# JuliaMolSim/Molly.jl

Hardware: AMD Instinct MI355X
Metric: ns_per_day (higher is better)
Workload: dtype f32; 1 GPU; 1M-atom LJ fluid (argon, rho=21.1/nm3), cubic PBC, DistanceCutoff 1.0 nm, r_list 1.2 nm, dt 2 fs, VelocityVerlet, remove_CM_motion=1; integrator=vv, n_atoms=1000000, rebuild_every=10, parallelism=single domain, block_atoms=256, j_split=2, pairs_half_list=75841147

## Files before the change

### molly.jl_amd/csrc/engine.hip

```cpp
#include <algorithm>
#include <chrono>
#include <cstddef>
#include <cstdlib>
#include <cstring>
#include <limits>
#include <memory>
#include <new>
#include <string>
#include <vector>

#include <unistd.h>

#include "bonded.h"
#include "stochastic.h"
#include "constraints.h"
#include "virtual_sites.h"
#include "pme.h"
#include "step_fused.h"
#include "hilbert.h"
#include "kernels.h"
#include "list_policy.h"
#include "replan.h"
#include "halo_step.h"
#include "forces_launch.h"
// ... 742 lines not shown
        bool step = false;
        bool gcv = false;
        bool cm = false, measure = false;
        double dt = 0;
        const StochP<T>* lang = nullptr;
        bool halo = false, halo_cm_in = false;
        bool fuse_spread = false, fuse_terms = false;
        const double* cm_sum_in = nullptr;
        T4* frc = nullptr;
    };
    struct PassRes {
        bool step = false; int parts = 0;
        bool gs = false, spread = false, terms = false;
        bool cm_summed = false;
    };
    bool packed_kind(bool energy) const {
        return std::is_same<T, float>::value && ljm == LJ_DIST_UNIFORM && coulm == MHIP_COUL_NONE && !energy && !minimg && n_special == 0 && eshift == ESHIFT_SCALED && I.lj_c12 != T(0);
    }
    int packed_stride(int tile_max, bool energy) const {
        if (!packed_kind(energy) || segmented) return 0;
        for (int k = 0; k < 3; ++k) if (tile_max + 1 < SOA_STRIDES[k]) return SOA_STRIDES[k];
        return 0;
    }
    PassRes launch_pair_kernel(bool energy, int part = 0, bool allow_gs = false, const PassReq& req = PassReq{}) {
        PassRes res;
        prune_resolve(!(xf_direct && n_ghost > 0));
        ForceArgs<T> A;
        A.G = G; A.I = I; A.n_owned = n_owned; A.BI = BI; A.BI_shift = ilog2(BI); A.JS = JS; A.T_cap = T_cap; A.T_lds = tile_lds; A.R_cap = R_cap;
        A.n_blocks = n_blocks; A.blocks_per_xcd = cdiv(n_blocks, 8);
        A.orig = nullptr; A.S = StochP<T>{};
        A.pos = pos[cur].p; A.lj = lj[cur].p; A.tile_idx = tile_idx.p; A.tile_cnt = tile_cnt.p;
        if constexpr (std::is_same<T, float>::value) {
            if (dual && !inner_valid && !energy && allow_gs && part == 0 && !req.frc && adopt_env && gs_groups() > 0 && cnt_outer_valid && margin_zero && !(lp.skin_in < lp.skin)
                && lp.last_outer_step == pass_step && n_ghost == 0 && !host_prune) adopt_outer_list();
        }
        const bool use_inner = dual && inner_valid;
        const bool prune = dual && !inner_valid && !energy;
        const int GS = gs_groups();
        if constexpr (std::is_same<T, float>::value) {
            if (allow_gs && GS > 0 && use_inner && !energy && part == 0 && gs_list_id == n_filters && !req.frc) {
                const int q_lds = (max_tile_in + GS - 1) / GS + 1;
                if (gs_lds_bytes(q_lds, BI, JS / GS) <= (size_t)MAX_LDS_BYTES / GS) {
                    frc_parts.reserve((size_t)(GS - 1) * cap);
                    GsArgs Z;
                    Z.G = G; Z.I = I; Z.n_owned = n_owned; Z.BI = BI; Z.BI_shift = ilog2(BI); Z.JS = JS; Z.GS = GS; Z.lgGS = ilog2(GS); Z.R_cap = GS * R_cap;
                     Z.T_cap = T_cap; Z.Q_lds = q_lds;
// ... 17 lines not shown
                                                  reinterpret_cast<const BondedArgs<float>&>(static_cast<const BondedArgs<T>&>(bonded.slot_args(G, I, pos[cur].p, inv.p))), cdiv(bonded.n_blocks(), 4), lds, stream,
                                                  gs_cm_fin ? pending_cm.parts_arg() : (const double*)nullptr, pending_cm.n, gs_cm_fin ? cm_fin_buf.p : (double*)nullptr);
                        if (gs_cm_fin) pending_cm.moved(cm_fin_buf.p, 1);
                        res.spread = with_spread; res.terms = !with_spread;
                    } else launch_forces_gs(Z, coulm, minimg, stream);
                    prof.end(0, stream);
                    MHIP_HIP(hipGetLastError());
                    ++n_force_calls; ++n_gs_passes; res.gs = true;
                    if (Z.dbg && (n_gs_passes % stamps_every()) == 0) stamps_dump("", (size_t)n_blocks * GS * 4 * 8);
                    return res;
                }
            }
        }
        const size_t prune_extra = prune ? prune_lds_bytes(std::min(T_cap, max_tile + 1), BI * JS) + 16 : 0;
        carve_force_lds(use_inner ? max_tile_in : max_tile, prune_extra);
        last_pass_tile = use_inner ? max_tile_in : max_tile;
        A.T_lds = tile_lds;
        if (use_inner && !inner_is_outer) { A.tile_idx = tile_idx_in.p; A.tile_cnt = tile_cnt_in.p; }
        A.nbr = (use_inner && !inner_is_outer) ? nbr_in.p : nbr.p; A.wave_rows = (use_inner && !inner_is_outer) ? wave_rows_in.p : wave_rows.p;
        A.nbr_dst = nullptr; A.rows_dst = nullptr; A.pos_snap = nullptr; A.blk_disp2 = nullptr; A.r_prune2 = r_prune2;
        A.tile_idx_dst = nullptr; A.tile_cnt_dst = nullptr; A.mark_off = 0; A.snap_dst = nullptr; A.any_special = n_special > 0 ? 1 : 0; A.eshift = eshift;
        A.cnt_dst = nullptr;
        A.soa = packed_stride(use_inner ? max_tile_in : max_tile, energy);
        if (A.soa) lds_force = std::max((size_t)3 * A.soa * sizeof(float) + 64, (size_t)JS * 4 * BI * sizeof(T) + 32);
        A.part = 0; A.blk_ghost = nullptr;
        if (part != 0 && !prune) {
            DBuf<int32_t>& fl = use_inner ? blk_ghost_in : blk_ghost; bool& ok = use_inner ? ghost_flags_in_ok : ghost_flags_ok;
            if (!ok) {
                fl.reserve(n_blocks);
                hipLaunchKernelGGL(k_block_ghost_flags, dim3(n_blocks), dim3(WAVE), 0, stream, n_blocks, T_cap, n_owned, (const int32_t*)A.tile_idx, (const int32_t*)A.tile_cnt, fl.p);
                ok = true;
            }
            A.part = part; A.blk_ghost = fl.p;
        }
        if (prune) {
            wave_rows_in.reserve((size_t)n_blocks * JS * (BI / WAVE)); nbr_in.reserve((size_t)n_blocks * JS * R_cap * BI); blk_disp2.reserve((size_t)n_blocks * (BI / WAVE));
            A.nbr_dst = nbr_in.p; A.rows_dst = wave_rows_in.p; A.pos_snap = pos_snap.p; A.blk_disp2 = blk_disp2.p;
            pos_snap_in.reserve(cap);
            A.snap_dst = pos_snap_in.p;
            if (n_ghost > 0) MHIP_HIP(hipMemcpyAsync(pos_snap_in.p + n_owned, pos[cur].p + n_owned, (size_t)n_ghost * sizeof(T4), hipMemcpyDeviceToDevice, stream));
            lp.last_prune_step = pass_step;
            tile_idx_in.reserve((size_t)n_blocks * T_cap); tile_cnt_in.reserve(n_blocks);
            A.tile_idx_dst = tile_idx_in.p; A.tile_cnt_dst = tile_cnt_in.p;
            inner_is_outer = false;
            if (GS > 0) { cnt_in.reserve((size_t)n_blocks * JS * BI); A.cnt_dst = cnt_in.p; }
            A.mark_off = (int)((lds_force + 15) & ~(size_t)15);
            if (A.soa && A.mark_off != prune_mark_ct(A.soa)) throw ApiError{MHIP_ERR_STATE, "internal: the packed pruning pass expects its renumbering table at " + std::to_string(prune_mark_ct(A.soa)) + ", the carve-up put it at " + std::to_string(A.mark_off)};
            lds_force = (size_t)A.mark_off + prune_lds_bytes(tile_lds, BI * JS);
            if (lds_force > (size_t)MAX_LDS_BYTES) throw ApiError{MHIP_ERR_CAPACITY, "prune pass LDS carve-up exceeds 160 KiB"};
        }
        A.blk_center = blk_center.p; A.frc = req.frc ? req.frc : frc[cur].p; A.pe_part = red_part.p;
        A.cm_fin_in = nullptr; A.cm_fin_n = 0; A.cm_fin_out = nullptr;
        A.vel = nullptr; A.pos_next = nullptr; A.dt = T(0); A.dt2 = T(0); A.cm_in = nullptr; A.cm_n = 0; A.cm_pub = nullptr; A.step_seq = 0; A.cm_out = nullptr; A.trk_part = nullptr; A.snap_a = nullptr; A.snap_b = nullptr;
        const bool cm_fin = (in_vv_fused || in_lang_fused) && !energy && n_ghost == 0 && part == 0 && pending_cm.mode() == 2 && pending_cm.n > 1 && pending_cm.n <= 65536;
        if (cm_fin) { cm_fin_buf.reserve(4); A.cm_fin_in = pending_cm.parts_arg(); A.cm_fin_n = pending_cm.n; A.cm_fin_out = cm_fin_buf.p; }
        else if (req.cm_sum_in && !energy && n_ghost == 0 && part == 0) {
            cm_fin_buf.reserve(4); A.cm_fin_in = req.cm_sum_in; A.cm_fin_n = pending_cm.n; A.cm_fin_out = cm_fin_buf.p; res.cm_summed = true;
        }
        A.level_pairs = (prune && JS == 2) ? 1 : 0;
        A.dbg = (!prune && !energy) ? stamps_begin((size_t)n_blocks * 16 * 8) : nullptr;
        bool do_step = false;
        if constexpr (std::is_same<T, float>::value) {
            do_step = req.step && fuse_step_env && A.soa != 0 && use_inner && !prune && part == 0 && !req.frc && (n_ghost == 0 || req.halo) && pending_cm.mode() != 1;
            if (req.halo && !do_step) throw ApiError{MHIP_ERR_STATE, "internal: the fused ghosted step was asked for a pass that cannot integrate"};
            if (do_step) {
                pos_alt.reserve(cap); cm_blk.reserve(2 * 4 * (size_t)n_blocks + 8);
                if (!cm_pub.p) { cm_pub.reserve(4); MHIP_HIP(hipMemsetAsync(cm_pub.p, 0, 4 * sizeof(unsigned long long), stream)); }
                A.vel = vel[cur].p; A.pos_next = pos_alt.p; A.dt = T(req.dt); A.dt2 = T(req.dt) / T(2);
                A.cm_in = pending_cm.parts_arg(); A.cm_n = pending_cm.n; A.cm_pub = cm_pub.p; A.step_seq = ++step_seq;
                A.cm_out = req.cm ? cm_blk.p + (size_t)step_half * 4 * n_blocks : (double*)nullptr;
                A.trk_part = nullptr; A.snap_a = pos_snap_in.p; A.snap_b = pos_snap.p;
// ... 33 lines not shown
        prof.end(prune ? 4 : 0, stream);
        MHIP_HIP(hipGetLastError());
        ++n_force_calls;
        if (A.dbg && (n_force_calls % stamps_every()) == 0) stamps_report();
        if (prune) {
            const bool late = xf_direct && n_ghost > 0 && prune_late_env;
            if (late) { h_prune.make(N_FLAGS); ev_prune.make(hipEventDisableTiming); }
            int32_t* const h_dst = late ? h_prune : h_flags;
            hipLaunchKernelGGL(k_prune_summary, dim3(1), dim3(1024), 0, stream, n_blocks, n_blocks * JS * (BI / WAVE), n_blocks * (BI / WAVE), R_cap,
                               (const int32_t*)tile_cnt_in.p, wave_rows_in.p, (const float*)blk_disp2.p, flags.p, h_dst);
            if (n_ghost > 0) {
                hipLaunchKernelGGL(k_max_disp<T>, dim3(std::min(cdiv(n_ghost, 256), 1024)), dim3(256), 0, stream, n_ghost, (const T4*)pos[cur].p + n_owned, (const T4*)pos_snap.p + n_owned,
                                   reinterpret_cast<unsigned int*>(flags.p + FLAG_MAX_DISP2), G);
                MHIP_HIP(hipMemcpyAsync(h_dst, flags.p, N_FLAGS * sizeof(int32_t), hipMemcpyDeviceToHost, stream));
            }
            ++n_filters; ghost_flags_in_ok = false; lp.next_check_step = -1; hx.tile_ok = false; hx.trk_step = -1;
            inner_valid = true;
            if (late) {
                MHIP_HIP(hipEventRecord(ev_prune, stream));
                prune_pending = true; prune_pending_id = n_filters; prune_disp_exceeded = false;
                max_tile_in = max_tile;
            } else {
                MHIP_HIP(hipStreamSynchronize(stream));
                prune_pending = false;
                float d2; std::memcpy(&d2, &h_flags[FLAG_MAX_DISP2], sizeof(float));
                total_rows = h_flags[FLAG_TOTAL_ROWS]; max_tile_in = h_flags[FLAG_MAX_TILE];
                prune_disp_exceeded = !lp.prune_stands(std::sqrt((double)d2));
                if (debug_on) std::fprintf(stderr, "[mhip] prune: max disp %.5f nm (margin %.3f) rows %lld exceeded %d calls %lld\n", std::sqrt((double)d2), lp.prune_margin(), (long long)total_rows, (int)prune_disp_exceeded, (long long)n_force_calls);
            }
        }
        return res;
    }

    DBuf<double> cm_fin_buf;
    int step_half = 0;
    uint32_t step_seq = 0;
    int64_t n_fused_steps = 0;
    int step_parts = 0;
    const bool fuse_gcv_env = env_int("MOLLYHIP_FUSE_GATHER_VV", 1) != 0;
    DBuf<T4> pos_alt; DBuf<double> cm_blk; DBuf<unsigned long long> cm_pub;
    const bool fuse_step_env = env_int("MOLLYHIP_FUSE_STEP", 1) != 0;
    const bool halo_waiter_env = env_int("MOLLYHIP_HALO_WAITER", 1) != 0;
    const bool prune_late_env = env_int("MOLLYHIP_PRUNE_LATE", 1) != 0;
    bool packed_step_possible() {
        if (!fuse_step_env || !dual || !inner_valid || stale || !packed_kind(false)) return false;
        prune_resolve(false);
        if (prune_pending && max_tile_in + 1 >= SOA_STRIDES[2]) prune_resolve(true);
        if (max_tile_in + 1 >= SOA_STRIDES[2]) return false;
        carve_force_lds(max_tile_in);
        return packed_stride(max_tile_in, false) != 0;
    }
// ... 1820 lines not shown
```

### molly.jl_amd/csrc/kernels.h

```cpp
#pragma once
#include <type_traits>
#include "physics.h"
#include "halo_xfer.h"
#include "philox.h"

namespace mhip {

enum { FLAG_MINIMG = 0, FLAG_OVERFLOW = 1, FLAG_MAX_TILE = 2, FLAG_MAX_ROWS = 3, FLAG_NAN = 4, FLAG_TOTAL_ROWS = 5, FLAG_MAX_CELLS = 6, FLAG_MAX_DISP2 = 7, FLAG_MAX_V2 = 8, N_FLAGS = 10 };
enum { OVF_TILE = 1, OVF_ROWS = 2, OVF_BOXCELLS = 4, OVF_SLOT = 8 };

constexpr int MAX_BOX_CELLS = 8192;
constexpr uint32_t XL_EXCLUDED = 1u << 30, XL_SPECIAL = 1u << 31, XL_INDEX = (1u << 30) - 1u;

constexpr int ESHIFT_SCALED = 2;
constexpr int SLOT_MAX_SCALED = 16383;
__host__ __device__ inline uint32_t entry_slot(uint32_t e, int sh) { return sh ? (e >> sh) : (e & 0x7fffu); }
__host__ __device__ inline uint32_t entry_special(uint32_t e, int sh) { return sh ? 0u : (e >> 15); }
__host__ __device__ inline uint32_t make_entry(uint32_t slot, uint32_t sp, int sh) { return sh ? (slot << sh) : (slot | (sp << 15)); }

template <class T> __device__ inline int cell_coord(T x, int d, const GridP<T>& G) {
    T rel = G.periodic[d] ? x : x - G.origin[d];
    int c = (int)M<T>::floor(rel * G.inv_cs[d]);
    return min(max(c, 0), G.nc[d] - 1);
}

extern "C" __device__ int mhip_writelane_i32(int src, int lane, int old) __asm("llvm.amdgcn.writelane.i32");
__device__ inline void mask_to_lane(int& lo, int& hi, unsigned long long mask, int dst) {
// ... 1086 lines not shown
#pragma unroll
    for (int o = 32; o > 0; o >>= 1) for (int c = 0; c < 4; ++c) a[c] += __shfl_xor(a[c], o, 64);
    if ((threadIdx.x & 63) == 0) for (int c = 0; c < 4; ++c) sh_pub[threadIdx.x >> 6][c] = a[c];
    __syncthreads();
    if (threadIdx.x < 3) {
        double t = 0, m = 0;
        for (int q = 0; q < (int)(blockDim.x >> 6); ++q) { t += sh_pub[q][threadIdx.x]; m += sh_pub[q][3]; }
        const float vc = (float)(t / m);
        __hip_atomic_store(&pub[threadIdx.x], (unsigned long long)__float_as_uint(vc) | ((unsigned long long)seq << 32), __ATOMIC_RELAXED, __HIP_MEMORY_SCOPE_AGENT);
    }
}
[[maybe_unused]] static __device__ inline void cm_finalize_in_block(const double* __restrict__ part, int n_part, double* out4, unsigned char* smem) {
    double a[4] = {0, 0, 0, 0};
    for (int q = threadIdx.x; q < n_part; q += blockDim.x) { const double* p = part + 4 * (int64_t)q; a[0] += p[0]; a[1] += p[1]; a[2] += p[2]; a[3] += p[3]; }
#pragma unroll
    for (int o = 32; o > 0; o >>= 1) for (int c = 0; c < 4; ++c) a[c] += __shfl_xor(a[c], o, 64);
    double* sh = reinterpret_cast<double*>(smem);
    if ((threadIdx.x & 63) == 0) for (int c = 0; c < 4; ++c) sh[4 * (threadIdx.x >> 6) + c] = a[c];
    __syncthreads();
    if (threadIdx.x < 4) { double t = 0; for (int q = 0; q < (int)(blockDim.x >> 6); ++q) t += sh[4 * q + threadIdx.x]; out4[threadIdx.x] = t; }
    __syncthreads();
}
constexpr int SOA_STRIDES[3] = {2049, 3073, 4097};
__host__ __device__ constexpr int prune_mark_ct(int soa) { return (3 * soa * 4 + 64 + 15) & ~15; }
__host__ __device__ inline size_t prune_lds_bytes(int t_seg, int nthr) { return (size_t)(((t_seg + 8) & ~7) * 2) + ((size_t)nthr + 4) * 4 + 8 * 8 * 4 + ((size_t)nthr + 64) * 4 + 16 * 8 + 32; }

#ifndef MHIP_FAST_MIN_WAVES
#define MHIP_FAST_MIN_WAVES 8
#endif
#ifndef MHIP_SB
#define MHIP_SB 4
#endif
template <class T, int LJM, int COULM, bool ENERGY, bool MINIMG, bool SEG, bool PRUNE>
constexpr int force_min_waves() { return (std::is_same<T, float>::value && LJM == LJ_DIST_UNIFORM && COULM == MHIP_COUL_NONE && !ENERGY && !MINIMG && !SEG && !PRUNE) ? MHIP_FAST_MIN_WAVES : 1; }

template <class T, int LJM, int COULM, bool ENERGY, bool MINIMG, bool SEG, bool PRUNE, int SOA_STRIDE = 4097, bool STEP = false, bool HALO = false, bool LANG = false>
__global__ void __launch_bounds__(BlockLimits<T>::max_threads, (force_min_waves<T, LJM, COULM, ENERGY, MINIMG, SEG, PRUNE>()))
k_forces(ForceArgs<T> A) {
    static_assert(!HALO || (STEP && std::is_same<T, float>::value), "the ghosted form exists for the fused fp32 step only");
    static_assert(!LANG || (STEP && !HALO), "the Langevin update rides in the fused single-domain step only");
    using T4 = typename Vec<T>::T4;
    using T2 = typename Vec<T>::T2;
    constexpr bool PER_ATOM_LJ = (LJM == LJ_DIST || LJM == LJ_GENERIC);
    extern __shared__ __align__(32) unsigned char smem[];
    const GridP<T>& G = A.G;
    int wg = blockIdx.x;
    if constexpr (STEP) {
        if (wg == 0) {
            if constexpr (HALO) { if (A.cm_in) halo_cm_publish(A.H, A.cm_pub, A.step_seq, smem); }
            else if (A.cm_in) step_cm_publish(A.cm_in, A.cm_n, A.cm_pub, A.step_seq, smem);
            return;
        }
        --wg;
    }
    int b = (wg & 7) * A.blocks_per_xcd + (wg >> 3);
    [[maybe_unused]] int hflags = 0;
    if constexpr (HALO) { b = A.H.order[wg]; if (b < 0) return; hflags = A.H.flags[b]; }
// ... 41 lines not shown
    int rows = 0;
    bool own_done = false;
    auto own_ready = [&]() {
        if (own_done) return;
        own_done = true;
        if constexpr (NO_TRI) pi = localise(pi_raw, std::false_type{});
        else pi = tri_local ? localise(pi_raw, std::true_type{}) : localise(pi_raw, std::false_type{});
        lji = pre_e(lji_raw);
        rows = __builtin_amdgcn_readfirstlane(rows_lane);
    };
    if constexpr (PRUNE) own_ready();
    const uint2* my_rows = A.nbr + (((int64_t)b * A.JS + js) * A.R_cap) * A.BI + li;
    const int32_t* tix = (HALO ? A.H.tsrc : A.tile_idx) + (int64_t)b * A.T_cap;
    if constexpr (HALO) { if (hflags & 1) halo_wait_block(A.H); }
    T fx = T(0), fy = T(0), fz = T(0), pe = T(0);
    [[maybe_unused]] T vir[6] = {T(0), T(0), T(0), T(0), T(0), T(0)};
    uint64_t acc = 0;
    int kept = 0;
    uint2* out_rows = nullptr;
    if constexpr (PRUNE) out_rows = A.nbr_dst + (((int64_t)b * A.JS + js) * A.R_cap) * A.BI + li;
    [[maybe_unused]] uint16_t* l_new = nullptr; [[maybe_unused]] int32_t* l_scan = nullptr; [[maybe_unused]] float* l_box = nullptr;
    [[maybe_unused]] int32_t* l_cnt = nullptr; [[maybe_unused]] int32_t* l_wmax = nullptr; [[maybe_unused]] const uint2* l_lut = nullptr;
    [[maybe_unused]] int n_new = 0;
    if constexpr (PRUNE) {
        l_new = reinterpret_cast<uint16_t*>(smem + A.mark_off);
        l_scan = reinterpret_cast<int32_t*>(smem + A.mark_off + ((A.T_lds + 8) & ~7) * 2);
        l_box = reinterpret_cast<float*>(l_scan + nthr + 4);
        l_wmax = reinterpret_cast<int32_t*>(l_box + 64); l_cnt = l_wmax + 64;
        if (tid < 64) l_wmax[tid] = 0;
        l_lut = reinterpret_cast<const uint2*>(l_cnt + nthr);
        if (tid < 16) {
            uint32_t sel[2] = {0x0c0c0c0cu, 0x0c0c0c0cu};
            int p = 0;
            for (int j = 0; j < 4; ++j) if ((tid >> j) & 1) {
                const int sh = (p & 1) * 16;
                sel[p >> 1] = (sel[p >> 1] & ~(0xffffu << sh)) | ((uint32_t)((2 * j) | ((2 * j + 1) << 8)) << sh);
                ++p;
            }
            reinterpret_cast<uint2*>(l_cnt + nthr)[tid] = make_uint2(sel[0], sel[1]);
        }
        const int lpb = A.BI >> 3;
        float mn[3] = {(float)pi.x, (float)pi.y, (float)pi.z}, mx[3] = {(float)pi.x, (float)pi.y, (float)pi.z};
        for (int o = lpb >> 1; o > 0; o >>= 1)
#pragma unroll
            for (int d = 0; d < 3; ++d) { mn[d] = fminf(mn[d], __shfl_xor(mn[d], o, WAVE)); mx[d] = fmaxf(mx[d], __shfl_xor(mx[d], o, WAVE)); }
        if (js == 0 && (li & (lpb - 1)) == 0) {
            reinterpret_cast<float4*>(l_box)[(li / lpb) * 2] = make_float4(mn[0], mn[1], mn[2], 0.f);
            reinterpret_cast<float4*>(l_box)[(li / lpb) * 2 + 1] = make_float4(mx[0], mx[1], mx[2], 0.f);
        }
        if (A.snap_dst && js == 0 && valid) A.snap_dst[si] = pi_raw;
    }
    [[maybe_unused]] auto emit4 = [&](uint32_t n0, uint32_t n1, uint32_t n2, uint32_t n3, bool k0, bool k1, bool k2, bool k3) {
        const uint32_t m = (k0 ? 1u : 0u) | (k1 ? 2u : 0u) | (k2 ? 4u : 0u) | (k3 ? 8u : 0u);
        const uint2 sel = l_lut[m];
        const uint32_t x = __builtin_amdgcn_perm(n1, n0, 0x05040100u), y = __builtin_amdgcn_perm(n3, n2, 0x05040100u);
        const uint64_t p = ((uint64_t)__builtin_amdgcn_perm(y, x, sel.y) << 32) | __builtin_amdgcn_perm(y, x, sel.x);
        const int np = kept & 3, sh = np * 16;
        const uint64_t c_lo = acc | (p << sh), c_hi = (p >> 1) >> (63 - sh);
        const int cnt = __builtin_popcount(m);
        const bool flush = np + cnt >= 4;
        if (flush) out_rows[(int64_t)(kept >> 2) * A.BI] = make_uint2((uint32_t)c_lo, (uint32_t)(c_lo >> 32));
        acc = flush ? c_hi : c_lo;
        kept += cnt;
    };
    auto emit = [&](uint32_t e) {
        const int np = kept & 3;
        acc |= (uint64_t)e << (np * 16);
        if (np == 3) { out_rows[(int64_t)(kept >> 2) * A.BI] = make_uint2((uint32_t)acc, (uint32_t)(acc >> 32)); acc = 0; }
        ++kept;
    };

    constexpr bool FAST_CT = std::is_same<T, float>::value && LJM == LJ_DIST_UNIFORM && COULM == MHIP_COUL_NONE && !ENERGY && !MINIMG && !SEG;
    const int seg_cap = A.T_lds;
// ... 11 lines not shown
                    for (int k = 0; k < SB; ++k) s[k] = tix[min(t0 + k * nthr + tid, A.T_cap - 1)];
#pragma unroll
                    for (int k = 0; k < SB; ++k) {
                        s[k] = (t0 + k * nthr + tid < n_here) ? s[k] : (int)((int64_t)b * A.BI);
                        if constexpr (HALO) {
                            if (s[k] >= 0) p[k] = A.pos[s[k]];
                            else { const float* gr = A.H.rows + 3 * (size_t)(-1 - s[k]); p[k] = make4<T>((T)peer_row_load(gr), (T)peer_row_load(gr + 1), (T)peer_row_load(gr + 2), T(0)); }
                        } else p[k] = A.pos[s[k]];
                    }
#pragma unroll
                    for (int k = 0; k < SB; ++k) {
                        const int t = t0 + k * nthr + tid;
                        if (t < n_here) {
                            const T4 pl = localise(p[k], tri_tag);
                            if (packed3) { l_p3[t] = (float)pl.x; l_p3[SOA_STRIDE + t] = (float)pl.y; l_p3[2 * SOA_STRIDE + t] = (float)pl.z; }
                            else l_pos[t] = pl;
                        }
                    }
                };
                round(0);
                for (int t0 = SB * nthr; t0 < n_here; t0 += SB * nthr) round(t0);
                return;
            }
            for (int t0 = 0; t0 < n_here; t0 += SB * nthr) {
                int s[SB]; T4 p[SB]; [[maybe_unused]] T2 q[SB];
                constexpr bool GUARD = !(FAST_CT && !PRUNE);
                const int kmax = GUARD ? min(SB, (n_here - t0 + nthr - 1) / nthr) : SB;
#pragma unroll
                for (int k = 0; k < SB; ++k) {
                    if (k < kmax) {
                        const int t = min(t0 + k * nthr + tid, n_here - 1);
                        s[k] = tix[seg_lo + t];
                    }
                }
#pragma unroll
                for (int k = 0; k < SB; ++k) if (k < kmax) { p[k] = A.pos[s[k]]; if constexpr (PER_ATOM_LJ) q[k] = A.lj[s[k]]; }
#pragma unroll
                for (int k = 0; k < SB; ++k) {
                    const int t = t0 + k * nthr + tid;
                    if (k < kmax && t < n_here) {
                        const T4 pl = localise(p[k], tri_tag);
                        if (packed3) { l_p3[t] = (float)pl.x; l_p3[SOA_STRIDE + t] = (float)pl.y; l_p3[2 * SOA_STRIDE + t] = (float)pl.z; }
                        else l_pos[t] = pl;
                        if constexpr (PER_ATOM_LJ) l_lj[t] = pre_e(q[k]);
                    }
                }
            }
        };
        if constexpr (NO_TRI) stage(std::false_type{});
        else { if (tri_local) stage(std::true_type{}); else stage(std::false_type{}); }
        own_ready();
        if (tid == 0) {
            if (packed3) { l_p3[n_here] = 1e4f; l_p3[SOA_STRIDE + n_here] = 1e4f; l_p3[2 * SOA_STRIDE + n_here] = 1e4f; }
            else l_pos[n_here] = make4<T>(T(1e4), T(1e4), T(1e4), T(0));
            if constexpr (PER_ATOM_LJ) l_lj[n_here] = make2<T>(T(0), T(0));
        }
        __syncthreads();
        if constexpr (PRUNE) {
            constexpr int NW = 8;
            const float reach2 = (float)A.r_prune2 * 1.001f + 1e-12f;
            const float bL[3] = {(float)G.L[0], (float)G.L[1], (float)G.L[2]}, biL[3] = {(float)G.invL[0], (float)G.invL[1], (float)G.invL[2]};
            auto stays = [&](int t) -> bool {
                if constexpr (MINIMG) { if (G.triclinic) return true; }
                float p[3];
                if (packed3) { p[0] = l_p3[t]; p[1] = l_p3[SOA_STRIDE + t]; p[2] = l_p3[2 * SOA_STRIDE + t]; }
                else { const T4 q = l_pos[t]; p[0] = (float)q.x; p[1] = (float)q.y; p[2] = (float)q.z; }
                float best = 3.0e38f;
#pragma unroll 1
                for (int w = 0; w < NW; ++w) {
                    const float4 lo = reinterpret_cast<const float4*>(l_box)[2 * w], hi = reinterpret_cast<const float4*>(l_box)[2 * w + 1];
                    float ex, ey, ez;
                    if constexpr (MINIMG) {
                        const float blo[3] = {lo.x, lo.y, lo.z}, bhi[3] = {hi.x, hi.y, hi.z};
                        float e[3];
#pragma unroll
                        for (int d = 0; d < 3; ++d) {
                            float dd = p[d] - 0.5f * (blo[d] + bhi[d]);
                            if (G.periodic[d]) dd -= bL[d] * rintf(dd * biL[d]);
                            e[d] = fmaxf(fabsf(dd) - 0.5f * (bhi[d] - blo[d]) - 1e-5f * bL[d], 0.f);
                        }
                        ex = e[0]; ey = e[1]; ez = e[2];
                    } else {
                        ex = fmaxf(fmaxf(lo.x - p[0], p[0] - hi.x), 0.f); ey = fmaxf(fmaxf(lo.y - p[1], p[1] - hi.y), 0.f); ez = fmaxf(fmaxf(lo.z - p[2], p[2] - hi.z), 0.f);
                    }
                    best = fminf(best, ex * ex + ey * ey + ez * ez);
                }
                return best <= reach2;
            };
            const int per = (n_here + nthr - 1) / nthr, t0 = min(tid * per, n_here), t1 = min(t0 + per, n_here);
            int cnt = 0;
            uint32_t keep_bits = 0;
            for (int t = t0; t < t1; ++t) { const bool k = stays(t); cnt += k ? 1 : 0; if (t - t0 < 32) keep_bits |= (k ? 1u : 0u) << (t - t0); }
            l_scan[tid] = cnt;
            __syncthreads();
            if (tid < WAVE) {
                int run = 0;
                for (int base = 0; base < nthr; base += WAVE) {
                    int v = (base + tid < nthr) ? l_scan[base + tid] : 0, x = v;
#pragma unroll
                    for (int o = 1; o < WAVE; o <<= 1) { int u = __shfl_up(x, o, WAVE); if (tid >= o) x += u; }
                    if (base + tid < nthr) l_scan[base + tid] = run + x - v;
                    run += __shfl(x, WAVE - 1, WAVE);
                }
                if (tid == 0) l_scan[nthr] = run;
            }
            __syncthreads();
            {
                int run = n_new + l_scan[tid];
                for (int t = t0; t < t1; ++t) {
                    if ((t - t0 < 32) ? ((keep_bits >> (t - t0)) & 1u) != 0u : stays(t)) { l_new[t] = (uint16_t)(packed3 ? run << ESHIFT_SCALED : run); A.tile_idx_dst[(int64_t)b * A.T_cap + run] = tix[seg_lo + t]; ++run; }
                    else l_new[t] = (uint16_t)0xffffu;
                }
            }
            n_new += l_scan[nthr];
            __syncthreads();
        }
        stamp(1);
        auto walk_rows = [&](auto spec_tag) {
            constexpr bool SPEC = decltype(spec_tag)::value;
            if constexpr (FAST_CT && !SPEC) { if (packed3) {
                typedef float v2f __attribute__((ext_vector_type(2)));
                const v2f pix = {(float)pi.x, (float)pi.x}, piy = {(float)pi.y, (float)pi.y}, piz = {(float)pi.z, (float)pi.z};
                const float c6 = (float)A.I.lj_c6, c12 = (float)A.I.lj_c12, rc2 = (float)A.I.lj_rc2, rp2 = (float)A.r_prune2;
                const float rc2n = __int_as_float(__float_as_int(rc2) + 1);
                const v2f cut_a = {-0x1p100f, -0x1p100f}, cut_b = {rc2n * 0x1p100f, rc2n * 0x1p100f};
                const v2f c48v = {c12, c12}, c24v = {c6, c6};
                v2f fx2 = {(float)fx, 0.f}, fy2 = {(float)fy, 0.f}, fz2 = {(float)fz, 0.f};
                typedef __attribute__((address_space(3))) const char* lds_cptr;
                const lds_cptr lbase = (lds_cptr)(uintptr_t)0;
                auto lds3 = [&](uint32_t oa, uint32_t ob, v2f& dx, v2f& dy, v2f& dz) {
                    typedef __attribute__((address_space(3))) const float* lds_fptr;
                    const lds_fptr pa = (lds_fptr)(lbase + oa), pb = (lds_fptr)(lbase + ob);
                    dx = (v2f){pa[0], pb[0]} - pix; dy = (v2f){pa[SOA_STRIDE], pb[SOA_STRIDE]} - piy; dz = (v2f){pa[2 * SOA_STRIDE], pb[2 * SOA_STRIDE]} - piz;
                };
                auto row = [&](const uint2 e4) {
                    const uint32_t oa = e4.x & 0xffffu, ob = e4.x >> 16, oc = e4.y & 0xffffu, od = e4.y >> 16;
                    v2f dx0, dy0, dz0, dx1, dy1, dz1;
                    lds3(oa, ob, dx0, dy0, dz0); lds3(oc, od, dx1, dy1, dz1);
                    __builtin_amdgcn_sched_group_barrier(0x100, 12, 0);
                    const v2f r20 = __builtin_elementwise_fma(dz0, dz0, __builtin_elementwise_fma(dy0, dy0, dx0 * dx0));
                    const v2f r21 = __builtin_elementwise_fma(dz1, dz1, __builtin_elementwise_fma(dy1, dy1, dx1 * dx1));
                    if constexpr (PRUNE) {
                        typedef __attribute__((address_space(3))) const unsigned short* lds_hptr;
                        auto new_entry = [&](uint32_t o) -> uint32_t { return (uint32_t)*(lds_hptr)(lbase + prune_mark_ct(SOA_STRIDE) + (o >> 1)); };
                        const uint32_t na = new_entry(oa), nb = new_entry(ob), nc = new_entry(oc), nd = new_entry(od);
                        emit4(na, nb, nc, nd, r20.x <= rp2, r20.y <= rp2, r21.x <= rp2, r21.y <= rp2);
                    }
                    const float t0 = __builtin_amdgcn_rcpf(r20.x * r20.y), t1 = __builtin_amdgcn_rcpf(r21.x * r21.y);
                    const v2f u0 = (v2f){r20.y, r20.x} * t0, u1 = (v2f){r21.y, r21.x} * t1;
                    v2f in0, in1;
                    asm("v_pk_fma_f32 %0, %1, %2, %3 clamp\n\ts_nop 0" : "=v"(in0) : "v"(r20), "s"(cut_a), "v"(cut_b));
                    asm("v_pk_fma_f32 %0, %1, %2, %3 clamp\n\ts_nop 0" : "=v"(in1) : "v"(r21), "s"(cut_a), "v"(cut_b));
                    const v2f q0 = u0 * u0, q1 = u1 * u1;
                    const v2f w0 = u0 * in0, w1 = u1 * in1;
                    const v2f c0 = q0 * u0, c1 = q1 * u1;
                    const v2f g0 = __builtin_elementwise_fma(c0, c48v, -c24v), g1 = __builtin_elementwise_fma(c1, c48v, -c24v);
                    const v2f h0 = c0 * w0, h1 = c1 * w1;
                    const v2f f0 = g0 * h0, f1 = g1 * h1;
                    fx2 -= dx0 * f0; fy2 -= dy0 * f0; fz2 -= dz0 * f0;
                    fx2 -= dx1 * f1; fy2 -= dy1 * f1; fz2 -= dz1 * f1;
                };
                if (rows > 0) {
                    const int last = rows - 1;
                    constexpr int D = 2;
                    uint2 e[D] = {my_rows[0], my_rows[(int64_t)min(1, last) * A.BI]};
                    auto next = [&](int q) -> uint2 { return my_rows[(int64_t)min(q, last) * A.BI]; };
                    int r = 0;
                    for (; r + D <= rows; r += D) {
#pragma unroll
// ... 94 lines not shown
            __syncthreads();
            const int kp = l_cnt[tid ^ A.BI], total = kept + kp, mine = js == 0 ? (total + 1) >> 1 : total >> 1;
            if (kept > mine) {
                uint16_t* to = reinterpret_cast<uint16_t*>(A.nbr_dst + (((int64_t)b * A.JS + (js ^ 1)) * A.R_cap) * A.BI + li);
                const uint16_t* from = reinterpret_cast<const uint16_t*>(out_rows);
                for (int q = 0; q < kept - mine; ++q) {
                    const int ps = mine + q, pd = kp + q;
                    to[(((int64_t)(pd >> 2) * A.BI) << 2) + (pd & 3)] = from[(((int64_t)(ps >> 2) * A.BI) << 2) + (ps & 3)];
                }
            }
            kept = mine;
        }
        if (A.cnt_dst) A.cnt_dst[((int64_t)b * A.JS + js) * A.BI + li] = (uint16_t)min(kept, 65535);
        atomicMax(&l_wmax[js * NWB + (li >> 6)], (kept + 3) >> 2);
        __syncthreads();
        const int rows_wave = l_wmax[js * NWB + (li >> 6)];
        if (level) {
            uint16_t* mine16 = reinterpret_cast<uint16_t*>(out_rows);
            for (int p2 = kept; p2 < 4 * rows_wave; ++p2) mine16[(((int64_t)(p2 >> 2) * A.BI) << 2) + (p2 & 3)] = (uint16_t)SENTP;
        } else
        while (((kept + 3) >> 2) < rows_wave || (kept & 3)) emit(SENTP);
        if (tid < A.JS * NWB) A.rows_dst[b * A.JS * NWB + tid] = l_wmax[tid];
        if (tid == 0) A.tile_cnt_dst[b] = n_new;
        float d2 = 0.f;
        if (valid && js == 0) {
            T4 q = A.pos_snap[si];
            T ex = pi_raw.x - q.x, ey = pi_raw.y - q.y, ez = pi_raw.z - q.z;
            disp_image(ex, ey, ez, G);
            d2 = (float)(ex * ex + ey * ey + ez * ez);
        }
        d2 = wave_max(d2);
        if (js == 0 && (tid & 63) == 0) A.blk_disp2[b * (A.BI >> 6) + (li >> 6)] = d2;
    }
    stamp(2);
    [[maybe_unused]] T4 st_v, st_p;
    [[maybe_unused]] int64_t se = 0;
    [[maybe_unused]] unsigned long long st_w[3] = {0, 0, 0};
    [[maybe_unused]] int snd0 = 0, snd1 = 0;
    if constexpr (STEP) {
        __builtin_amdgcn_s_setprio(3);
        se = step_atom();
        if constexpr (HALO) { if ((hflags & 2) && js == 0 && se < A.n_owned) { snd0 = A.H.snd_start[se]; snd1 = A.H.snd_start[se + 1]; } }
        if (js == 0 && se < A.n_owned) {
            st_v = A.vel[se]; st_p = A.pos[se];
            if (A.cm_in) {
#pragma unroll
                for (int c = 0; c < 3; ++c) st_w[c] = __hip_atomic_load(&A.cm_pub[c], __ATOMIC_RELAXED, __HIP_MEMORY_SCOPE_AGENT);
            }
        }
    }
    if (A.JS > 1) {
        __syncthreads();
// ... 79 lines not shown
            }
            if (A.trk_part && tid < 3) { float mm = 0.f; for (int q = 0; q < 4 * nw; ++q) mm = fmaxf(mm, shf[4 * q + tid]); A.trk_part[(int64_t)tid * A.n_blocks + b] = mm; }
        }
        if (mine) { A.vel[se] = v; A.pos_next[se] = p; }
        if constexpr (HALO) {
            if (js == 0) {
                if (hflags & 2) {
                    if (!(hflags & 1)) { const int ln = tid & 63; if (ln < A.H.n_peers && !xfer_wait(&A.H.seq_in[A.H.peers[ln]], A.H.seq_wait, A.H.err, A.H.ticks, (9 << 8) | A.H.peers[ln])) atomicOr(A.H.err, 1); }
                    if (mine) for (int r = snd0; r < snd1; ++r) {
                        const HaloSend e = A.H.snd[r];
                        float* d = e.dst + (int64_t)A.H.parity_send * A.H.half_stride;
                        __hip_atomic_store(d, (float)p.x + e.sx, __ATOMIC_RELAXED, __HIP_MEMORY_SCOPE_SYSTEM);
                        __hip_atomic_store(d + 1, (float)p.y + e.sy, __ATOMIC_RELAXED, __HIP_MEMORY_SCOPE_SYSTEM);
                        __hip_atomic_store(d + 2, (float)p.z + e.sz, __ATOMIC_RELAXED, __HIP_MEMORY_SCOPE_SYSTEM);
                    }
                }
                asm volatile("s_waitcnt vmcnt(0)" ::: "memory");
                unsigned int before = 0;
                if ((tid & 63) == 0) before = __hip_atomic_fetch_add(A.H.done, 1u, __ATOMIC_RELAXED, __HIP_MEMORY_SCOPE_AGENT);
                before = (unsigned int)__builtin_amdgcn_readfirstlane((int)before);
                if (before == A.H.n_done - 1u) halo_tail(A.H, A.cm_out, A.n_blocks);
            }
        }
    } else {
        if (js == 0 && valid) A.frc[si] = make4<T>(fx, fy, fz, T(0));
    }
    stamp(3);
    if constexpr (!ENERGY) {
        if (A.cm_fin_out && wg == 0) { __syncthreads(); cm_finalize_in_block(A.cm_fin_in, A.cm_fin_n, A.cm_fin_out, smem); }
    }
    if constexpr (ENERGY) {
        if (A.JS > 1) {
            T* red = reinterpret_cast<T*>(smem);
#pragma unroll
            for (int half = 0; half < 2; ++half) {
                __syncthreads();
#pragma unroll
                for (int c = 0; c < 3; ++c) red[(js * 4 + c) * A.BI + li] = vir[3 * half + c];
                __syncthreads();
                if (js == 0) for (int q = 1; q < A.JS; ++q) for (int c = 0; c < 3; ++c) vir[3 * half + c] += red[(q * 4 + c) * A.BI + li];
            }
        }
        __syncthreads();
        double* dred = reinterpret_cast<double*>(smem);
        for (int c = 0; c < 7; ++c) {
            if (js == 0) dred[li] = valid ? 0.5 * (double)(c == 0 ? pe : vir[c - 1]) : 0.0;
// ... 339 lines not shown
```

Measured before the change: 1372 ns/day.

## Compact pruning pass staging to a smaller LDS stride with box-distance filtering

Result: faster. 1413 ns/day (median of 6 runs) (+3.0%).

```diff
diff --git a/molly.jl_amd/csrc/engine.hip b/molly.jl_amd/csrc/engine.hip
--- a/molly.jl_amd/csrc/engine.hip
+++ b/molly.jl_amd/csrc/engine.hip
@@ -788,6 +788,11 @@
         for (int k = 0; k < 3; ++k) if (tile_max + 1 < SOA_STRIDES[k]) return SOA_STRIDES[k];
         return 0;
     }
+    int prune_kept_tile = -1;
+    static int prune_stride_for(int tile, int soa_outer) {
+        for (int k = 0; k < 3; ++k) if (tile + 1 < SOA_STRIDES[k]) return std::min(SOA_STRIDES[k], soa_outer);
+        return soa_outer;
+    }
     PassRes launch_pair_kernel(bool energy, int part = 0, bool allow_gs = false, const PassReq& req = PassReq{}) {
         PassRes res;
         prune_resolve(!(xf_direct && n_ghost > 0));
@@ -851,6 +856,9 @@
         A.tile_idx_dst = nullptr; A.tile_cnt_dst = nullptr; A.mark_off = 0; A.snap_dst = nullptr; A.any_special = n_special > 0 ? 1 : 0; A.eshift = eshift;
         A.cnt_dst = nullptr;
         A.soa = packed_stride(use_inner ? max_tile_in : max_tile, energy);
+        const bool prune_sync = prune && n_ghost == 0;
+        const int soa_outer = A.soa;
+        if (prune && A.soa && prune_sync && GS <= 0 && prune_kept_tile >= 0) A.soa = prune_stride_for(prune_kept_tile + prune_kept_tile / 128 + 4, soa_outer);
         if (A.soa) lds_force = std::max((size_t)3 * A.soa * sizeof(float) + 64, (size_t)JS * 4 * BI * sizeof(T) + 32);
         A.part = 0; A.blk_ghost = nullptr;
         if (part != 0 && !prune) {
@@ -875,7 +883,7 @@
             if (GS > 0) { cnt_in.reserve((size_t)n_blocks * JS * BI); A.cnt_dst = cnt_in.p; }
             A.mark_off = (int)((lds_force + 15) & ~(size_t)15);
             if (A.soa && A.mark_off != prune_mark_ct(A.soa)) throw ApiError{MHIP_ERR_STATE, "internal: the packed pruning pass expects its renumbering table at " + std::to_string(prune_mark_ct(A.soa)) + ", the carve-up put it at " + std::to_string(A.mark_off)};
-            lds_force = (size_t)A.mark_off + prune_lds_bytes(tile_lds, BI * JS);
+            lds_force = A.soa ? prune_lds_total(A.soa, tile_lds, BI * JS) : (size_t)A.mark_off + prune_lds_bytes(tile_lds, BI * JS);
             if (lds_force > (size_t)MAX_LDS_BYTES) throw ApiError{MHIP_ERR_CAPACITY, "prune pass LDS carve-up exceeds 160 KiB"};
         }
         A.blk_center = blk_center.p; A.frc = req.frc ? req.frc : frc[cur].p; A.pe_part = red_part.p;
@@ -955,11 +963,25 @@
                 max_tile_in = max_tile;
             } else {
                 MHIP_HIP(hipStreamSynchronize(stream));
+                while (A.soa && prune_compacts(A.soa) && h_flags[FLAG_MAX_TILE] > A.soa - 1) {
+                    if (debug_on) std::fprintf(stderr, "[mhip] prune: a compacted tile of %d atoms outgrew stride %d, pass repeated\n", (int)h_flags[FLAG_MAX_TILE], A.soa);
+                    A.soa = prune_stride_for(h_flags[FLAG_MAX_TILE], soa_outer);
+                    A.mark_off = prune_mark_ct(A.soa);
+                    lds_force = prune_lds_total(A.soa, tile_lds, BI * JS);
+                    prof.begin(4, stream);
+                    launch_forces_any(A, energy);
+                    prof.end(4, stream);
+                    MHIP_HIP(hipGetLastError());
+                    hipLaunchKernelGGL(k_prune_summary, dim3(1), dim3(1024), 0, stream, n_blocks, n_blocks * JS * (BI / WAVE), n_blocks * (BI / WAVE), R_cap,
+                                       (const int32_t*)tile_cnt_in.p, wave_rows_in.p, (const float*)blk_disp2.p, flags.p, h_dst);
+                    MHIP_HIP(hipStreamSynchronize(stream));
+                }
+                prune_kept_tile = h_flags[FLAG_MAX_TILE];
                 prune_pending = false;
                 float d2; std::memcpy(&d2, &h_flags[FLAG_MAX_DISP2], sizeof(float));
                 total_rows = h_flags[FLAG_TOTAL_ROWS]; max_tile_in = h_flags[FLAG_MAX_TILE];
                 prune_disp_exceeded = !lp.prune_stands(std::sqrt((double)d2));
-                if (debug_on) std::fprintf(stderr, "[mhip] prune: max disp %.5f nm (margin %.3f) rows %lld exceeded %d calls %lld\n", std::sqrt((double)d2), lp.prune_margin(), (long long)total_rows, (int)prune_disp_exceeded, (long long)n_force_calls);
+                if (debug_on) std::fprintf(stderr, "[mhip] prune: max disp %.5f nm (margin %.3f) rows %lld exceeded %d calls %lld tile %d of %d stride %d lds %zu\n", std::sqrt((double)d2), lp.prune_margin(), (long long)total_rows, (int)prune_disp_exceeded, (long long)n_force_calls, max_tile_in, max_tile, A.soa, lds_force);
             }
         }
         return res;
diff --git a/molly.jl_amd/csrc/kernels.h b/molly.jl_amd/csrc/kernels.h
--- a/molly.jl_amd/csrc/kernels.h
+++ b/molly.jl_amd/csrc/kernels.h
@@ -3,6 +3,7 @@
 #include "physics.h"
 #include "halo_xfer.h"
 #include "philox.h"
+#include "prune_lds.h"
 
 namespace mhip {
 
@@ -1135,17 +1136,21 @@
     __syncthreads();
 }
 constexpr int SOA_STRIDES[3] = {2049, 3073, 4097};
-__host__ __device__ constexpr int prune_mark_ct(int soa) { return (3 * soa * 4 + 64 + 15) & ~15; }
-__host__ __device__ inline size_t prune_lds_bytes(int t_seg, int nthr) { return (size_t)(((t_seg + 8) & ~7) * 2) + ((size_t)nthr + 4) * 4 + 8 * 8 * 4 + ((size_t)nthr + 64) * 4 + 16 * 8 + 32; }
+static_assert(PRUNE_OUTER_STRIDE == SOA_STRIDES[2], "prune_lds.h and the packed loop disagree about the largest stride");
 
 #ifndef MHIP_FAST_MIN_WAVES
 #define MHIP_FAST_MIN_WAVES 8
+#endif
+#ifndef MHIP_PRUNE_MIN_WAVES
+#define MHIP_PRUNE_MIN_WAVES 6
 #endif
 #ifndef MHIP_SB
 #define MHIP_SB 4
 #endif
 template <class T, int LJM, int COULM, bool ENERGY, bool MINIMG, bool SEG, bool PRUNE>
-constexpr int force_min_waves() { return (std::is_same<T, float>::value && LJM == LJ_DIST_UNIFORM && COULM == MHIP_COUL_NONE && !ENERGY && !MINIMG && !SEG && !PRUNE) ? MHIP_FAST_MIN_WAVES : 1; }
+constexpr int force_min_waves() {
+    return (std::is_same<T, float>::value && LJM == LJ_DIST_UNIFORM && COULM == MHIP_COUL_NONE && !ENERGY && !MINIMG && !SEG) ? (PRUNE ? MHIP_PRUNE_MIN_WAVES : MHIP_FAST_MIN_WAVES) : 1;
+}
 
 template <class T, int LJM, int COULM, bool ENERGY, bool MINIMG, bool SEG, bool PRUNE, int SOA_STRIDE = 4097, bool STEP = false, bool HALO = false, bool LANG = false>
 __global__ void __launch_bounds__(BlockLimits<T>::max_threads, (force_min_waves<T, LJM, COULM, ENERGY, MINIMG, SEG, PRUNE>()))
@@ -1233,11 +1238,17 @@
     [[maybe_unused]] uint16_t* l_new = nullptr; [[maybe_unused]] int32_t* l_scan = nullptr; [[maybe_unused]] float* l_box = nullptr;
     [[maybe_unused]] int32_t* l_cnt = nullptr; [[maybe_unused]] int32_t* l_wmax = nullptr; [[maybe_unused]] const uint2* l_lut = nullptr;
     [[maybe_unused]] int n_new = 0;
+    constexpr bool P_FAST = PRUNE && std::is_same<T, float>::value && LJM == LJ_DIST_UNIFORM && COULM == MHIP_COUL_NONE && !ENERGY && !MINIMG && !SEG;
+    [[maybe_unused]] bool p_compact = false;
+    [[maybe_unused]] float p_d2 = 0.f;
+    [[maybe_unused]] constexpr uint32_t P_SENT = (uint32_t)(SOA_STRIDE - 1) << ESHIFT_SCALED;
+    if constexpr (P_FAST) p_compact = !A.any_special && A.soa == SOA_STRIDE && A.eshift == ESHIFT_SCALED;
     if constexpr (PRUNE) {
         l_new = reinterpret_cast<uint16_t*>(smem + A.mark_off);
-        l_scan = reinterpret_cast<int32_t*>(smem + A.mark_off + ((A.T_lds + 8) & ~7) * 2);
-        l_box = reinterpret_cast<float*>(l_scan + nthr + 4);
+        l_scan = reinterpret_cast<int32_t*>(smem + A.mark_off + prune_table_bytes(A.T_lds));
+        l_box = reinterpret_cast<float*>((P_FAST && prune_compacts(SOA_STRIDE) && p_compact) ? l_scan : l_scan + nthr + 4);
         l_wmax = reinterpret_cast<int32_t*>(l_box + 64); l_cnt = l_wmax + 64;
+        if constexpr (P_FAST) { if (prune_compacts(SOA_STRIDE) && p_compact) l_scan = l_cnt; }
         if (tid < 64) l_wmax[tid] = 0;
         l_lut = reinterpret_cast<const uint2*>(l_cnt + nthr);
         if (tid < 16) {
@@ -1260,6 +1271,15 @@
             reinterpret_cast<float4*>(l_box)[(li / lpb) * 2 + 1] = make_float4(mx[0], mx[1], mx[2], 0.f);
         }
         if (A.snap_dst && js == 0 && valid) A.snap_dst[si] = pi_raw;
+        if constexpr (P_FAST) {
+            if (valid && js == 0) {
+                T4 q = A.pos_snap[si];
+                T ex = pi_raw.x - q.x, ey = pi_raw.y - q.y, ez = pi_raw.z - q.z;
+                disp_image(ex, ey, ez, G);
+                p_d2 = (float)(ex * ex + ey * ey + ez * ez);
+            }
+            if (p_compact) __syncthreads();
+        }
     }
     [[maybe_unused]] auto emit4 = [&](uint32_t n0, uint32_t n1, uint32_t n2, uint32_t n3, bool k0, bool k1, bool k2, bool k3) {
         const uint32_t m = (k0 ? 1u : 0u) | (k1 ? 2u : 0u) | (k2 ? 4u : 0u) | (k3 ? 8u : 0u);
@@ -1317,6 +1337,58 @@
                 for (int t0 = SB * nthr; t0 < n_here; t0 += SB * nthr) round(t0);
                 return;
             }
+            if constexpr (P_FAST) { if (p_compact) {
+                constexpr int PS = PRUNE_SUB;
+                const int nwv = nthr >> 6, wv = tid >> 6, lane = tid & 63;
+                const float reach2 = (float)A.r_prune2 * 1.001f + 1e-12f;
+                int half = 0;
+                for (int t0 = 0; t0 < n_here; t0 += PS * nthr, half ^= 1) {
+                    int s[PS]; T4 p[PS]; float best[PS];
+                    const int kmax = min(PS, (n_here - t0 + nthr - 1) / nthr);
+#pragma unroll
+                    for (int k = 0; k < PS; ++k) if (k < kmax) s[k] = tix[min(t0 + k * nthr + tid, n_here - 1)];
+#pragma unroll
+                    for (int k = 0; k < PS; ++k) if (k < kmax) p[k] = A.pos[s[k]];
+#pragma unroll
+                    for (int k = 0; k < PS; ++k) { best[k] = 3.0e38f; if (k < kmax) p[k] = localise(p[k], tri_tag); }
+#pragma unroll 1
+                    for (int w = 0; w < 8; ++w) {
+                        const float4 lo = reinterpret_cast<const float4*>(l_box)[2 * w], hi = reinterpret_cast<const float4*>(l_box)[2 * w + 1];
+#pragma unroll
+                        for (int k = 0; k < PS; ++k) if (k < kmax) {
+                            const float px = (float)p[k].x, py = (float)p[k].y, pz = (float)p[k].z;
+                            const float ex = fmaxf(fmaxf(lo.x - px, px - hi.x), 0.f), ey = fmaxf(fmaxf(lo.y - py, py - hi.y), 0.f), ez = fmaxf(fmaxf(lo.z - pz, pz - hi.z), 0.f);
+                            best[k] = fminf(best[k], ex * ex + ey * ey + ez * ez);
+                        }
+                    }
+                    int* const wtot = l_scan + half * (PS * nwv);
+                    int rank[PS]; bool keep[PS];
+#pragma unroll
+                    for (int k = 0; k < PS; ++k) {
+                        keep[k] = false; rank[k] = 0;
+                        if (k < kmax) {
+                            keep[k] = t0 + k * nthr + tid < n_here && best[k] <= reach2;
+                            const unsigned long long m = __ballot(keep[k]);
+                            if (lane == 0) wtot[k * nwv + wv] = __popcll(m);
+                            rank[k] = __popcll(m & ((1ull << lane) - 1ull));
+                        }
+                    }
+                    __syncthreads();
+#pragma unroll
+                    for (int k = 0; k < PS; ++k) if (k < kmax) {
+                        int dst = n_new + rank[k], tot = 0;
+                        for (int w = 0; w < nwv; ++w) { const int c = wtot[k * nwv + w]; if (w < wv) dst += c; tot += c; }
+                        const int t = t0 + k * nthr + tid;
+                        if (keep[k]) {
+                            if (dst < SOA_STRIDE - 1) { l_p3[dst] = (float)p[k].x; l_p3[SOA_STRIDE + dst] = (float)p[k].y; l_p3[2 * SOA_STRIDE + dst] = (float)p[k].z; }
+                            A.tile_idx_dst[(int64_t)b * A.T_cap + dst] = s[k];
+                            l_new[t] = (uint16_t)((uint32_t)min(dst, SOA_STRIDE - 1) << ESHIFT_SCALED);
+                        } else if (t < n_here) l_new[t] = (uint16_t)P_SENT;
+                        n_new += tot;
+                    }
+                }
+                return;
+            } }
             for (int t0 = 0; t0 < n_here; t0 += SB * nthr) {
                 int s[SB]; T4 p[SB]; [[maybe_unused]] T2 q[SB];
                 constexpr bool GUARD = !(FAST_CT && !PRUNE);
@@ -1346,20 +1418,24 @@
         else { if (tri_local) stage(std::true_type{}); else stage(std::false_type{}); }
         own_ready();
         if (tid == 0) {
-            if (packed3) { l_p3[n_here] = 1e4f; l_p3[SOA_STRIDE + n_here] = 1e4f; l_p3[2 * SOA_STRIDE + n_here] = 1e4f; }
+            if (P_FAST && p_compact) {
+                l_p3[SOA_STRIDE - 1] = 1e4f; l_p3[2 * SOA_STRIDE - 1] = 1e4f; l_p3[3 * SOA_STRIDE - 1] = 1e4f;
+                l_new[n_here] = (uint16_t)P_SENT;
+            }
+            else if (packed3) { l_p3[n_here] = 1e4f; l_p3[SOA_STRIDE + n_here] = 1e4f; l_p3[2 * SOA_STRIDE + n_here] = 1e4f; }
             else l_pos[n_here] = make4<T>(T(1e4), T(1e4), T(1e4), T(0));
             if constexpr (PER_ATOM_LJ) l_lj[n_here] = make2<T>(T(0), T(0));
         }
         __syncthreads();
-        if constexpr (PRUNE) {
+        if constexpr (PRUNE) { if (!(P_FAST && p_compact)) {
+            static_assert(!PRUNE || FAST_CT == P_FAST, "the packed pruning walk requires the compacting staging");
             constexpr int NW = 8;
             const float reach2 = (float)A.r_prune2 * 1.001f + 1e-12f;
             const float bL[3] = {(float)G.L[0], (float)G.L[1], (float)G.L[2]}, biL[3] = {(float)G.invL[0], (float)G.invL[1], (float)G.invL[2]};
             auto stays = [&](int t) -> bool {
                 if constexpr (MINIMG) { if (G.triclinic) return true; }
                 float p[3];
-                if (packed3) { p[0] = l_p3[t]; p[1] = l_p3[SOA_STRIDE + t]; p[2] = l_p3[2 * SOA_STRIDE + t]; }
-                else { const T4 q = l_pos[t]; p[0] = (float)q.x; p[1] = (float)q.y; p[2] = (float)q.z; }
+                { const T4 q = l_pos[t]; p[0] = (float)q.x; p[1] = (float)q.y; p[2] = (float)q.z; }
                 float best = 3.0e38f;
 #pragma unroll 1
                 for (int w = 0; w < NW; ++w) {
@@ -1403,13 +1479,13 @@
             {
                 int run = n_new + l_scan[tid];
                 for (int t = t0; t < t1; ++t) {
-                    if ((t - t0 < 32) ? ((keep_bits >> (t - t0)) & 1u) != 0u : stays(t)) { l_new[t] = (uint16_t)(packed3 ? run << ESHIFT_SCALED : run); A.tile_idx_dst[(int64_t)b * A.T_cap + run] = tix[seg_lo + t]; ++run; }
+                    if ((t - t0 < 32) ? ((keep_bits >> (t - t0)) & 1u) != 0u : stays(t)) { l_new[t] = (uint16_t)run; A.tile_idx_dst[(int64_t)b * A.T_cap + run] = tix[seg_lo + t]; ++run; }
                     else l_new[t] = (uint16_t)0xffffu;
                 }
             }
             n_new += l_scan[nthr];
             __syncthreads();
-        }
+        } }
         stamp(1);
         auto walk_rows = [&](auto spec_tag) {
             constexpr bool SPEC = decltype(spec_tag)::value;
@@ -1429,17 +1505,21 @@
                     dx = (v2f){pa[0], pb[0]} - pix; dy = (v2f){pa[SOA_STRIDE], pb[SOA_STRIDE]} - piy; dz = (v2f){pa[2 * SOA_STRIDE], pb[2 * SOA_STRIDE]} - piz;
                 };
                 auto row = [&](const uint2 e4) {
-                    const uint32_t oa = e4.x & 0xffffu, ob = e4.x >> 16, oc = e4.y & 0xffffu, od = e4.y >> 16;
+                    uint32_t oa = e4.x & 0xffffu, ob = e4.x >> 16, oc = e4.y & 0xffffu, od = e4.y >> 16;
+                    if constexpr (PRUNE) {
+                        typedef __attribute__((address_space(3))) const unsigned short* lds_hptr;
+                        auto new_entry = [&](uint32_t o) -> uint32_t { return (uint32_t)*(lds_hptr)(lbase + prune_mark_ct(SOA_STRIDE) + (o >> 1)); };
+                        const uint32_t na = new_entry(oa), nb = new_entry(ob), nc = new_entry(oc), nd = new_entry(od);
+                        __builtin_amdgcn_sched_group_barrier(0x100, 4, 0);
+                        oa = na; ob = nb; oc = nc; od = nd;
+                    }
                     v2f dx0, dy0, dz0, dx1, dy1, dz1;
                     lds3(oa, ob, dx0, dy0, dz0); lds3(oc, od, dx1, dy1, dz1);
                     __builtin_amdgcn_sched_group_barrier(0x100, 12, 0);
                     const v2f r20 = __builtin_elementwise_fma(dz0, dz0, __builtin_elementwise_fma(dy0, dy0, dx0 * dx0));
                     const v2f r21 = __builtin_elementwise_fma(dz1, dz1, __builtin_elementwise_fma(dy1, dy1, dx1 * dx1));
                     if constexpr (PRUNE) {
-                        typedef __attribute__((address_space(3))) const unsigned short* lds_hptr;
-                        auto new_entry = [&](uint32_t o) -> uint32_t { return (uint32_t)*(lds_hptr)(lbase + prune_mark_ct(SOA_STRIDE) + (o >> 1)); };
-                        const uint32_t na = new_entry(oa), nb = new_entry(ob), nc = new_entry(oc), nd = new_entry(od);
-                        emit4(na, nb, nc, nd, r20.x <= rp2, r20.y <= rp2, r21.x <= rp2, r21.y <= rp2);
+                        emit4(oa, ob, oc, od, r20.x <= rp2, r20.y <= rp2, r21.x <= rp2, r21.y <= rp2);
                     }
                     const float t0 = __builtin_amdgcn_rcpf(r20.x * r20.y), t1 = __builtin_amdgcn_rcpf(r21.x * r21.y);
                     const v2f u0 = (v2f){r20.y, r20.x} * t0, u1 = (v2f){r21.y, r21.x} * t1;
@@ -1580,12 +1660,14 @@
         while (((kept + 3) >> 2) < rows_wave || (kept & 3)) emit(SENTP);
         if (tid < A.JS * NWB) A.rows_dst[b * A.JS * NWB + tid] = l_wmax[tid];
         if (tid == 0) A.tile_cnt_dst[b] = n_new;
-        float d2 = 0.f;
-        if (valid && js == 0) {
-            T4 q = A.pos_snap[si];
-            T ex = pi_raw.x - q.x, ey = pi_raw.y - q.y, ez = pi_raw.z - q.z;
-            disp_image(ex, ey, ez, G);
-            d2 = (float)(ex * ex + ey * ey + ez * ez);
+        float d2 = p_d2;
+        if constexpr (!P_FAST) {
+            if (valid && js == 0) {
+                T4 q = A.pos_snap[si];
+                T ex = pi_raw.x - q.x, ey = pi_raw.y - q.y, ez = pi_raw.z - q.z;
+                disp_image(ex, ey, ez, G);
+                d2 = (float)(ex * ex + ey * ey + ez * ez);
+            }
         }
         d2 = wave_max(d2);
         if (js == 0 && (tid & 63) == 0) A.blk_disp2[b * (A.BI >> 6) + (li >> 6)] = d2;
@@ -1711,6 +1793,9 @@
                 if (before == A.H.n_done - 1u) halo_tail(A.H, A.cm_out, A.n_blocks);
             }
         }
+    } else if constexpr (P_FAST) {
+        const int64_t sa = step_atom();
+        if (js == 0 && sa < A.n_owned) A.frc[sa] = make4<T>(fx, fy, fz, T(0));
     } else {
         if (js == 0 && valid) A.frc[si] = make4<T>(fx, fy, fz, T(0));
     }
diff --git a/molly.jl_amd/csrc/prune_lds.h b/molly.jl_amd/csrc/prune_lds.h
--- /dev/null
+++ b/molly.jl_amd/csrc/prune_lds.h
@@ -0,0 +1,30 @@
+#pragma once
+#include <cstddef>
+
+#if defined(__HIPCC__) || defined(__CUDACC__)
+#define MHIP_PLDS_HD __host__ __device__
+#else
+#define MHIP_PLDS_HD
+#endif
+
+namespace mhip {
+
+constexpr int PRUNE_OUTER_STRIDE = 4097;
+constexpr int PRUNE_SUB = 4;
+constexpr int PRUNE_LDS_PER_CU = 160 * 1024;
+
+MHIP_PLDS_HD constexpr int prune_mark_ct(int soa) { return (3 * soa * 4 + 64 + 15) & ~15; }
+MHIP_PLDS_HD constexpr int prune_table_bytes(int t_seg) { return ((t_seg + 8) & ~7) * 2; }
+MHIP_PLDS_HD constexpr size_t prune_lds_bytes(int t_seg, int nthr) {
+    return (size_t)prune_table_bytes(t_seg) + ((size_t)nthr + 4) * 4 + 8 * 8 * 4 + ((size_t)nthr + 64) * 4 + 16 * 8 + 32;
+}
+MHIP_PLDS_HD constexpr bool prune_compacts(int soa) { return soa != 0 && soa < PRUNE_OUTER_STRIDE; }
+MHIP_PLDS_HD constexpr size_t prune_lds_bytes_compact(int t_outer, int nthr) {
+    return (size_t)prune_table_bytes(t_outer) + 8 * 8 * 4 + ((size_t)nthr + 64) * 4 + 16 * 8 + 32;
+}
+MHIP_PLDS_HD constexpr size_t prune_lds_total(int soa, int t_outer, int nthr) {
+    return (size_t)prune_mark_ct(soa) + (prune_compacts(soa) ? prune_lds_bytes_compact(t_outer, nthr) : prune_lds_bytes(t_outer, nthr));
+}
+MHIP_PLDS_HD constexpr int prune_blocks_per_cu(size_t lds_bytes) { return lds_bytes == 0 ? 0 : (int)((size_t)PRUNE_LDS_PER_CU / lds_bytes); }
+
+}
```
